# algbio/founderblockgraphs

Hardware: AMD Instinct MI355X
Metric: MSA columns segmented/sec (higher is better)
Workload: dtype u32

## Files before the change

founderblockgraphs_amd/csrc/ctx.hip:

```cpp
#include "fbg_internal.h"
#include <chrono>
#include <stdarg.h>
#include <stdio.h>
#include <ctype.h>
#include <string.h>
#include <algorithm>
#include <atomic>
#include <thread>
#include <vector>

static std::string g_global_err;

int fbg_fail(fbg_ctx *ctx, int code, const char *fmt, ...)
{
    char buf[1024];
    va_list ap;
    va_start(ap, fmt);
    vsnprintf(buf, sizeof(buf), fmt, ap);
    va_end(ap);
    if (ctx) ctx->err = buf; else g_global_err = buf;
    return code;
}

int fbg_reserve(fbg_ctx *ctx, DevBuf &b, size_t bytes, std::vector<DevBuf *> *owner, bool accounted)
// ... 160 lines not shown
    {"no_aux_stream", &FbgOptions::no_aux_stream},
    {"rank_no_threshold", &FbgOptions::rank_no_threshold},
    {"dp_literal", &FbgOptions::dp_literal},
    {"dp_wave", &FbgOptions::dp_wave},
    {"dp_safe_window", &FbgOptions::dp_safe_window},
    {"dp_tile", &FbgOptions::dp_tile},
    {"pure_scan", &FbgOptions::pure_scan},
    {"gapped_rank", &FbgOptions::gapped_rank},
    {"part_tricks_off", &FbgOptions::part_tricks_off},
    {"msd_sample_bins", &FbgOptions::msd_sample_bins},
    {"msd_min_force", &FbgOptions::msd_min_force},
    {"msd_probe", &FbgOptions::msd_probe},
    {"msd_xcd", &FbgOptions::msd_xcd},
    {"rank_no_lean", &FbgOptions::rank_no_lean},
    {"no_stream_upload", &FbgOptions::no_stream_upload},
    {"span_scan", &FbgOptions::span_scan},
    {"span_key_flags", &FbgOptions::span_key_flags},
    {"span_slow_split", &FbgOptions::span_slow_split},
    {"poison", &FbgOptions::poison},
    {"dpw_matrix", &FbgOptions::dpw_matrix},
    {"dp_chain1", &FbgOptions::dp_chain1},
    {"msd_ext", &FbgOptions::msd_ext},
    {"rows_wave", &FbgOptions::rows_wave},
};

struct InfoKey { const char *name; int64_t (*get)(const fbg_ctx &); };
static const InfoKey g_info_keys[] = {
    {"grs_threshold", [](const fbg_ctx &c) -> int64_t { return c.grs_t; }},
    {"grs_redone", [](const fbg_ctx &c) -> int64_t { return (int64_t)c.grs_redone; }},
    {"dp_kind", [](const fbg_ctx &c) -> int64_t { return c.dp_kind; }},
    {"msd_decline", [](const fbg_ctx &c) -> int64_t { return c.diag.msd_decline; }},
    {"pass1_ahead", [](const fbg_ctx &c) -> int64_t { return c.diag.pass1_ahead; }},
    {"ext_pairs", [](const fbg_ctx &c) -> int64_t { return c.diag.ext_pairs; }},
    {"text_pairs", [](const fbg_ctx &c) -> int64_t { return c.diag.text_pairs; }},
    {"rank_lean_used", [](const fbg_ctx &c) -> int64_t { return c.diag.rank_lean_used; }},
    {"rank_lean_launched", [](const fbg_ctx &c) -> int64_t { return c.diag.rank_lean_launched; }},
    {"pairs_rb", [](const fbg_ctx &c) -> int64_t { return c.diag.pairs_rb; }},
    {"key_b", [](const fbg_ctx &c) -> int64_t { return c.key_b; }},
    {"key_K", [](const fbg_ctx &c) -> int64_t { return c.key_K; }},
    {"key_packed", [](const fbg_ctx &c) -> int64_t { return c.key_packed; }},
    {"key_compact", [](const fbg_ctx &c) -> int64_t { return c.key_compact; }},
    {"alloc_calls", [](const fbg_ctx &c) -> int64_t { return (int64_t)c.alloc_calls; }},
    {"alloc_us", [](const fbg_ctx &c) -> int64_t { return (int64_t)c.alloc_us; }},
    {"span_decline", [](const fbg_ctx &c) -> int64_t { return c.diag.sp_decline; }},
    {"span_key_flags_used", [](const fbg_ctx &c) -> int64_t { return c.ix.index_valid && c.ix.spanned() && c.ix.sp_key_flags_sorted; }},
    {"span_scan_used", [](const fbg_ctx &c) -> int64_t { return c.ix.index_valid && c.ix.spanned(); }},
    {"span_scan_work", [](const fbg_ctx &c) -> int64_t { return (int64_t)c.sp_work; }},
    {"span_groups", [](const fbg_ctx &c) -> int64_t { return (int64_t)c.sp_G; }},
    {"span_odd_groups", [](const fbg_ctx &c) -> int64_t { return (int64_t)c.sp_n_odd[0] + c.sp_n_odd[1] + c.sp_n_odd[2] + c.sp_n_odd[3]; }},
    {"span_irregular", [](const fbg_ctx &c) -> int64_t { return (int64_t)c.sp_n_irr; }},
    {"span_chain", [](const fbg_ctx &c) -> int64_t { return (int64_t)c.sp_chain_n; }},
    {"span_slow_groups", [](const fbg_ctx &c) -> int64_t { return (int64_t)c.sp_slow_n; }},
    {"index_kind", [](const fbg_ctx &c) -> int64_t { return !c.ix.index_valid ? -1 : c.ix.part_active ? 3 : c.ix.granked() ? 2 : c.ix.ranked() ? 1 : 0; }},
};

static void options_from_env(FbgOptions &o)
{
// ... 512 lines not shown
```

founderblockgraphs_amd/csrc/fbg_internal.h:

```cpp
#pragma once
#include <cstring>
#include <cstdlib>
#include <hip/hip_runtime.h>
#include <stdint.h>
#include <string>
#include <vector>
#include "../../include/fbg_hip.h"

#define FBG_WAVE 64

struct DevBuf {
    void *p = nullptr;
    size_t cap = 0;
    bool listed = false;
    template <class T> T *as() const { return reinterpret_cast<T *>(p); }
};

struct Stager {
    void *base = nullptr;
    size_t slot_bytes = 0;
    int nslots = 0;
    hipEvent_t *ev = nullptr;
    hipStream_t stream = nullptr;
};

struct StageTimer {
    hipEvent_t start = nullptr, stop = nullptr;
    bool recorded = false;
    int launches = 0;
};

struct FbgOptions {
    int64_t no_ranked = 0, no_packed = 0, force_wide = 0, full_keys = 0, no_msd_sort = 0, msd_min = -1, bp_min = -1,
            record_scatter = 0, lcp_text = 0, no_aux_stream = 0, rank_no_threshold = 0, dp_literal = 0, dp_wave = 0,
            dp_safe_window = 0, dp_tile = 0, pure_scan = 0, gapped_rank = 0, part_tricks_off = 0, msd_sample_bins = 0, msd_min_force = 0, msd_probe = 0, msd_xcd = -1, rank_no_lean = 0, no_stream_upload = 0,
            span_scan = 0, span_key_flags = 0, span_slow_split = 0, poison = 0, dpw_matrix = 0, dp_chain1 = 0, msd_ext = 1, rows_wave = 0;
};

enum class IndexKind { none, record, ranked, gapped, span };

struct IndexState {
    bool index_valid = false;
    IndexKind kind = IndexKind::none;
    bool ranked() const { return kind == IndexKind::ranked; }
    bool granked() const { return kind == IndexKind::gapped || kind == IndexKind::span; }
    bool spanned() const { return kind == IndexKind::span; }
    uint32_t *sa_ptr = nullptr;
    uint64_t *rk_keys = nullptr;
    int rk_b = 0, rk_key_bits = 0, rk_K = 0;
    int rk_layout = 0, rk_pb = 0;
    bool grs_flagged = false;
    bool sp_key_flags_sorted = false;
    bool msd_ext_valid = false;
    bool lcp_from_keys = false;
    bool grs_ties_done = false;
    uint32_t n_exc = 0;
    bool part_active = false;
    bool gpart = false;
    int part = 0, nparts = 1;
    uint64_t part_count = 0;
    uint64_t part_T = 0;
    uint32_t part_gmin = 0;
};

struct BuildDiag {
    int64_t msd_decline = -1;
    int pass1_ahead = 0;
    int64_t ext_pairs = -1, text_pairs = -1;
    int rank_lean_launched = 0;
    int rank_lean_used = 0;
    int pairs_rb = -1;
    int sp_decline = 0;
};

struct SortExtras {
    const uint64_t *ebits = nullptr;
    const uint32_t *payload = nullptr;
    bool key_flags = false;
};

struct MsdPlan;
struct fbg_ctx {
    int device = 0;
    FbgOptions opt;
    std::string err;
    hipStream_t stream = nullptr;
    bool own_stream = false;
    hipStream_t aux = nullptr;
    hipEvent_t aux_fork = nullptr, aux_join = nullptr;
    bool aux_pending = false;
    Stager stager;
// ... 40 lines not shown
    DevBuf xlist;
    DevBuf gmax, excol, xslot;
    DevBuf xbits;
    DevBuf exc_scratch;
    DevBuf exc;
    int grs_tricks_off = 0;
    uint32_t grs_ign_lo = 0, grs_ign_hi = 0;
    DevBuf gwin;
    DevBuf gbits;
    bool pairs_similar = false;
    bool grs_part_failed = false;
    uint32_t grs_t = 1;
    uint64_t grs_redone = 0;
    DevBuf sp_cells;
    DevBuf sp_flagT;
    DevBuf sp_cwin;
    DevBuf sp_tiles, sp_gstart, sp_gcol, sp_gflags, sp_rstart, sp_rid, sp_gplo, sp_gphi, sp_gval, sp_odd, sp_irr, sp_chain, sp_slow, sp_mins;
    uint32_t sp_chain_n = 0, sp_slow_n = 0;
    uint64_t sp_G = 0, sp_R = 0, sp_n_irr = 0, sp_work = 0;
    uint32_t sp_n_odd[4] = {0, 0, 0, 0}, sp_odd_cap = 0;

    DevBuf keysA, keysB, valsA, valsB, grp, flags, list, tie_list, big_groups, tmp, small, scalars;
    DevBuf msd_ext;
    DevBuf kargs;
    alignas(16) unsigned char kargs_host[512];
    DevBuf msd_w, msd_v;
    DevBuf dp_a, dp_b, dp_c, dp_d, dp_e, dp_f, dp_g, dp_h, io_a, io_b, io_c, io_d;
    DevBuf bt_up, bt_dep;
    DevBuf ps_a, ps_b, ps_c, ps_d, ps_e, ps_f, ps_g, ps_h;
};

int fbg_fail(fbg_ctx *ctx, int code, const char *fmt, ...);
#define FBG_HIP_TRY(ctx, expr)                                                              \
    do {                                                                                    \
        hipError_t e_ = (expr);                                                             \
        if (e_ != hipSuccess)                                                               \
            return fbg_fail((ctx), e_ == hipErrorOutOfMemory ? FBG_ERR_OOM : FBG_ERR_HIP,   \
                            "%s failed: %s (%s:%d)", #expr, hipGetErrorString(e_), __FILE__, \
                            __LINE__);                                                      \
    } while (0)
#define FBG_TRY(expr)                \
    do {                             \
        int rc_ = (expr);            \
        if (rc_ != FBG_OK) return rc_; \
    } while (0)

// ... 99 lines not shown
```

founderblockgraphs_amd/csrc/rank_common.h:

```cpp
#pragma once
#include "fbg_internal.h"
#include "text_cmp.h"

#define RS_TG 4

__device__ __forceinline__ uint32_t rs_key_lcp(uint64_t a, uint64_t c, int b, int key_bits)
{
    const uint64_t d = a ^ c;
    const uint32_t bits = (uint32_t)(__clzll((long long)d) - (64 - key_bits));
    const uint32_t inv_b = (65536u + (uint32_t)b - 1) / (uint32_t)b;
    return (bits * inv_b) >> 16;
}

struct RankArgs {
    uint32_t magic32;
    uint64_t magic64;
    uint64_t *keys;
    uint32_t *vals;
    uint64_t pmask;
    int pb;
    const uint8_t *T;
    uint64_t N, n;
    uint64_t Ntext;
    uint64_t own_lo, own_hi;
    int first_part, last_part;
    int part_mode;
    int values_only;
    uint32_t row_len;
    uint32_t g_min;
    int b, key_bits, K, reversed;
    uint32_t *gmax;
    uint32_t *cand;
    uint32_t *blk_count;
    uint32_t region;
    uint32_t *ties;
    uint32_t *tie_count;
    uint32_t tie_region;
    uint2 *pairs;
    int pair_codes;
    unsigned long long *pair_stats;
    uint32_t *pair_count;
    uint32_t *pm;
    uint32_t *big;
    unsigned long long *counters;
};

struct Slot {
    uint64_t key;
    uint64_t pos;
    uint32_t col;
    uint32_t rem;
};

__device__ __forceinline__ uint32_t rs_col_of_rem(const RankArgs &a, uint32_t rem)
{
    return rem == 0 ? (uint32_t)a.n : (a.reversed ? rem - 1 : (uint32_t)a.n - rem);
}
template <int L> struct PosT { typedef uint32_t type; };
template <> struct PosT<FBG_SLOTS_WIDE> { typedef uint64_t type; };
template <int L> __device__ __forceinline__ uint64_t rs_key(const RankArgs &a, uint64_t k) { return a.keys[k] >> a.pb; }
template <int L> __device__ __forceinline__ uint64_t rs_pos_of(const RankArgs &a, uint64_t w, uint32_t v)
{
    if (L == FBG_SLOTS_PACKED) return w & a.pmask;
    if (L == FBG_SLOTS_WIDE) return ((w & a.pmask) << 32) | v;
    return v;
}
template <int L> __device__ __forceinline__ uint64_t rs_pos(const RankArgs &a, uint64_t k)
{
// ... 159 lines not shown
    const uint32_t lp = has_prev ? min(min(rs_key_lcp(kp, key, a.b, a.key_bits), rem), mrp) : 0u;
    const uint32_t ln = has_next ? min(min(rs_key_lcp(key, kn, a.b, a.key_bits), rem), mrn) : 0u;
    const uint32_t g = max(lp, ln) + 1;
    if (g >= a.g_min || rem <= 64) rs_update(a, rs_col_of_rem(a, rem), g);
}


static inline int rs_layout(const KeyGeom &g) { return g.packed ? FBG_SLOTS_PACKED : g.wide ? FBG_SLOTS_WIDE : FBG_SLOTS_PAIRS; }

static inline void rs_args_init(fbg_ctx *ctx, RankArgs &a, uint64_t *keys, uint32_t *vals, uint64_t slots, int layout, int pb, int b,
                         int key_bits, int K)
{
    a.keys = keys; a.vals = vals; a.T = ctx->text.as<uint8_t>();
    a.pb = layout != FBG_SLOTS_PAIRS ? pb : 0; a.pmask = layout != FBG_SLOTS_PAIRS ? (1ull << pb) - 1 : 0;
    a.N = slots; a.Ntext = ctx->N; a.n = ctx->n; a.row_len = (uint32_t)(ctx->n + 1);
    a.own_lo = 0; a.own_hi = slots; a.first_part = a.last_part = 1; a.part_mode = 0; a.values_only = 0;
    a.magic32 = (uint32_t)((1ull << 32) / (ctx->n + 1));
    a.magic64 = ~0ull / (ctx->n + 1);
    a.b = b; a.key_bits = key_bits; a.K = K; a.reversed = ctx->reversed;
    a.gmax = ctx->gmax.as<uint32_t>();
    a.cand = nullptr; a.pm = nullptr; a.blk_count = nullptr; a.region = 0;
    a.ties = nullptr; a.tie_count = nullptr; a.tie_region = 0; a.pairs = nullptr; a.pair_count = nullptr; a.pair_codes = 0;
    a.pair_stats = nullptr;
    a.big = ctx->big_groups.as<uint32_t>();
    a.counters = ctx->scalars.as<unsigned long long>() + 32;
    a.g_min = 0;
}
```

founderblockgraphs_amd/csrc/rank_scan.hip:

```cpp
#include <algorithm>
#include <cstring>
#include <vector>
#include "fbg_internal.h"
#include "text_cmp.h"
#include <rocprim/rocprim.hpp>

#include "rank_common.h"

#define RS_ITEMS 4
#define RS_THREADS 256
#define RS_CHUNK (RS_THREADS * RS_ITEMS)

template <int L, bool PLAIN> __global__ __launch_bounds__(RS_THREADS) __attribute__((amdgpu_waves_per_eu(7, 8))) void k_rank_scan(RankArgs a)
{
    __shared__ uint64_t skey[RS_CHUNK + 2 * RS_HALO];
    __shared__ uint32_t srem[RS_CHUNK + 2 * RS_HALO];
    __shared__ uint16_t sq[RS_CHUNK];
    __shared__ uint32_t sqn, s_cand_n, s_tie_n;
    const int lane = threadIdx.x & 63;
    const uint64_t nchunks = (a.own_hi - a.own_lo + RS_CHUNK - 1) / RS_CHUNK;
    if (threadIdx.x == 0) { s_cand_n = 0; s_tie_n = 0; }
    uint64_t w[RS_ITEMS + 1];
    uint32_t v[RS_ITEMS + 1];
    const int my_i = RS_HALO + RS_ITEMS * (int)threadIdx.x;
// ... 174 lines not shown

#define RL_EV_LO 3
#define RL_EV_HI 60
#define RL_EV (RL_EV_HI - RL_EV_LO + 1)
#define RL_THREADS 256
#define RL_WAVES (RL_THREADS / 64)
#define RL_LIST 128

struct LeanArgs {
    const uint64_t *keys;
    const uint8_t *ext;
    uint64_t own_lo, own_hi;
    uint32_t per_wave, pmask;
    int pb;
    float inv_row_len, eps, one_minus_eps, near_end;
};

__device__ __forceinline__ uint32_t rl_from_next(uint32_t v) { return (uint32_t)__builtin_amdgcn_update_dpp(0, (int)v, 0x130, 0xf, 0xf, false); }
__device__ __forceinline__ uint32_t rl_lanes_below(unsigned long long m)
{
    return __builtin_amdgcn_mbcnt_hi((uint32_t)(m >> 32), __builtin_amdgcn_mbcnt_lo((uint32_t)m, 0u));
}

__device__ __attribute__((noinline)) void rl_noted(const RankArgs &a, const uint2 *list, uint32_t n, uint32_t *s_pair_n)
{
    const int lane = threadIdx.x & 63;
    uint32_t base = 0;
    if (lane == 0) base = atomicAdd(s_pair_n, n);
    base = __shfl(base, 0, 64);
    if ((uint32_t)lane < n && base + (uint32_t)lane < a.tie_region) a.pairs[(size_t)blockIdx.x * a.tie_region + base + lane] = list[lane];
}

__device__ __attribute__((noinline)) void rl_queued(const RankArgs &a, const uint32_t *list, uint32_t n, uint32_t *s_cand_n, uint32_t *s_tie_n)
{
    const int lane = threadIdx.x & 63;
    bool want_cand = false, want_tie = false;
    uint64_t k = 0;
    if ((uint32_t)lane < n) {
        k = list[lane];
        const int64_t base = (int64_t)k - RS_HALO;
        const int lo_i = (int)max((int64_t)0, (int64_t)a.own_lo - base);
        const int hi_i = (int)min((int64_t)(2 * RS_HALO + 1), (int64_t)a.own_hi - base);
        const RsWordView view{a.keys + base, &a, lo_i, hi_i};
        rank_scan_slow(a, view, RS_HALO, lo_i, hi_i, k, want_cand, want_tie);
    }
    rs_append(want_cand, s_cand_n, a.cand, a.region, (uint32_t)k);
    rs_append(want_tie, s_tie_n, a.ties, a.tie_region, (uint32_t)k);
}

template <class E> __device__ __forceinline__ void rl_shift(E *list, uint32_t &n)
{
    const int lane = threadIdx.x & 63;
    const uint32_t rest = n - 64;
    if ((uint32_t)lane < rest) { const E v = list[64 + lane]; list[lane] = v; }
    n = rest;
}

__global__ __launch_bounds__(RL_THREADS) __attribute__((amdgpu_waves_per_eu(8, 8))) void k_rank_scan_lean(const RankArgs *__restrict__ ap, LeanArgs f)
{
    __shared__ uint2 s_note[RL_WAVES][RL_LIST];
    __shared__ uint32_t s_queue[RL_WAVES][RL_LIST];
    __shared__ uint32_t s_cand_n, s_tie_n, s_pair_n;
    const int lane = threadIdx.x & 63;
    const int wv = __builtin_amdgcn_readfirstlane((int)(threadIdx.x >> 6));
    if (threadIdx.x == 0) { s_cand_n = 0; s_tie_n = 0; s_pair_n = 0; }
    __syncthreads();
    uint2 *my_note = s_note[wv];
    uint32_t *my_queue = s_queue[wv];
    uint32_t nn = 0, nq = 0;
    const uint32_t own_lo = (uint32_t)f.own_lo, own_hi = (uint32_t)f.own_hi;
    const uint32_t wlo = own_lo + ((uint32_t)blockIdx.x * RL_WAVES + (uint32_t)wv) * f.per_wave;
    const uint32_t whi = min(own_hi, wlo + f.per_wave);
    const unsigned long long EVM = ((1ull << (RL_EV_HI + 1)) - 1) & ~((1ull << RL_EV_LO) - 1);
    const unsigned long long RNG = ~(1ull << 63);
    const uint64_t *__restrict__ keys = f.keys;
    const uint8_t *__restrict__ ext = f.ext;
    auto row_slot = [&](uint32_t k0) -> uint32_t { return min(max(k0 - RL_EV_LO + (uint32_t)lane, own_lo), own_hi - 1); };
    uint64_t xnext = wlo < whi ? keys[row_slot(wlo)] : 0ull;
    uint32_t enext = ext && wlo < whi ? ext[row_slot(wlo)] : 0u;
    for (uint32_t k0 = wlo; k0 < whi; k0 += RL_EV) {
        const uint64_t x = xnext;
        const uint32_t ex = enext;
        if (k0 + RL_EV < whi) {
            const uint32_t kn = row_slot(k0 + RL_EV);
            xnext = keys[kn];
            if (ext) enext = ext[kn];
        }
        const uint32_t slot = k0 - RL_EV_LO + (uint32_t)lane;
// ... 23 lines not shown
                const unsigned long long LONG = TIE & ~(PH | (PH << 1));
                const unsigned long long ADJL = ((LONG >> 1) | (LONG << 1)) & ~TIE;
                SS = EVM & PH & ~(NE | (NE >> 1) | R1 | (R1 << 1) | (R2 << 1) | R2 | (R1 >> 1) | (E << 2) | (E >> 2));
                const unsigned long long QP = EVM & PH & ~SS;
                const unsigned long long RUN = R1 | (R1 << 1) | ((PH & R2) << 2) | ((PH >> 1) & R2);
                Q = QP | (QP << 1) | (EVM & (LONG | ADJL | (~TIE & (RUN | NE))));
            }
            if (SS) {
                uint32_t cx = 0, cy = 0;
                if (ext) {
                    const uint32_t d = (ex ^ rl_from_next(ex)) & 255u;
                    const uint32_t c = d ? (uint32_t)(__builtin_clz(d) - 24) >> 1 : 4u;
                    cx = c << 30; cy = (c >> 2) << 30;
                }
                if ((SS >> lane) & 1ull) my_note[nn + rl_lanes_below(SS)] = make_uint2((lo & f.pmask) | cx, (lo_n & f.pmask) | cy);
                nn += (uint32_t)__popcll(SS);
            }
            if (Q) {
                if ((Q >> lane) & 1ull) my_queue[nq + rl_lanes_below(Q)] = slot;
                nq += (uint32_t)__popcll(Q);
            }
        }
        while (nq >= 64) { rl_queued(*ap, my_queue, 64, &s_cand_n, &s_tie_n); rl_shift(my_queue, nq); }
        if (nn >= 64) { rl_noted(*ap, my_note, 64, &s_pair_n); rl_shift(my_note, nn); }
    }
    if (nn) rl_noted(*ap, my_note, nn, &s_pair_n);
    if (nq) rl_queued(*ap, my_queue, nq, &s_cand_n, &s_tie_n);
    __syncthreads();
    if (threadIdx.x == 0) { ap->blk_count[blockIdx.x] = s_cand_n; ap->tie_count[blockIdx.x] = s_tie_n; ap->pair_count[blockIdx.x] = s_pair_n; }
}

static bool rs_lean_setup(const RankArgs &a, int pb, unsigned blocks, LeanArgs *f)
{
    const uint64_t own = a.own_hi - a.own_lo, waves = (uint64_t)blocks * RL_WAVES;
    f->per_wave = (uint32_t)(((own + waves - 1) / waves + RL_EV - 1) / RL_EV * RL_EV);
    f->keys = a.keys; f->ext = nullptr; f->own_lo = a.own_lo; f->own_hi = a.own_hi; f->pmask = (uint32_t)a.pmask; f->pb = pb;
    const double L = (double)a.row_len;
    const double delta = (ldexp(1.0, pb - 25) + ldexp(1.0, pb - 22) + 2.0) / L + 1e-6;
    f->inv_row_len = (float)(1.0 / L);
    f->eps = (float)(2.0 * delta);
    f->one_minus_eps = 1.0f - f->eps;
    f->near_end = (float)(1.0 - 65.0 / L - delta);
    return 2.0 * delta < 0.01 && pb <= 31 && a.own_hi < (1ull << 31);
}

template <int L> __global__ __launch_bounds__(256) void k_tie_simple(RankArgs a)
{
    const uint32_t have = a.tie_count[blockIdx.x];
    if (have > a.tie_region) { if (threadIdx.x == 0) a.counters[1] = 1; return; }
    for (uint32_t e = threadIdx.x; e < have; e += blockDim.x) {
        const uint64_t h = a.ties[(size_t)blockIdx.x * a.tie_region + e];
        uint64_t key[RS_TG], pos[RS_TG];
// ... 99 lines not shown
    __syncthreads();
    if (threadIdx.x < 64 && sh[threadIdx.x]) atomicAdd(&hist[threadIdx.x], sh[threadIdx.x]);
    if (threadIdx.x == 0) {
        atomicAdd(&counters[2], (unsigned long long)sties);
        atomicAdd(&counters[3], (unsigned long long)min((uint64_t)256, N - (uint64_t)blockIdx.x * 1024 * 256));
    }
}

__global__ void k_count_unfilled(const uint32_t *__restrict__ gmax, uint64_t n, uint32_t g_min, int reversed,
                                 unsigned long long *__restrict__ counters)
{
    const uint64_t x = (uint64_t)blockIdx.x * blockDim.x + threadIdx.x;
    const uint64_t rem = reversed ? x + 1 : n - x;
    const bool miss = x < n && rem > 64 && gmax[x] < g_min;
    const unsigned long long mask = __ballot(miss);
    if ((threadIdx.x & 63) == 0 && mask) atomicAdd(&counters[1 + 3], (unsigned long long)__popcll(mask));
}

__global__ void k_cand_compact(const uint32_t *__restrict__ regions, const uint32_t *__restrict__ counts,
                               const uint32_t *__restrict__ offsets, uint32_t region, uint32_t *__restrict__ out)
{
    const uint32_t c = counts[blockIdx.x] < region ? counts[blockIdx.x] : region, o = offsets[blockIdx.x];
    for (uint32_t i = threadIdx.x; i < c; i += blockDim.x) out[o + i] = regions[(size_t)blockIdx.x * region + i];
}

#define RS_BIG_GROUPS 1024
#define RS_BIG_MEMBERS 8192
template <int L> __global__ void k_tie_groups(RankArgs a, uint64_t T, int by_list)
{
    const uint64_t t = (uint64_t)blockIdx.x * blockDim.x + threadIdx.x;
    if (t >= T) return;
    const uint64_t k0 = by_list ? (uint64_t)a.cand[t] : a.own_lo + t;
    const uint64_t key = rs_key<L>(a, k0);
    if (k0 > a.own_lo && rs_key<L>(a, k0 - 1) == key) return;
    if (k0 + 1 >= a.own_hi || rs_key<L>(a, k0 + 1) != key) return;
    uint32_t s = 1;
    while (k0 + s < a.own_hi && s <= RS_BIG_MEMBERS && rs_key<L>(a, k0 + s) == key) s++;
    if (s > 64) {
        if (s > RS_BIG_MEMBERS) { a.counters[1] = 1; return; }
        const unsigned long long e = atomicAdd(&a.counters[5], 1ull);
        if (e >= RS_BIG_GROUPS) { a.counters[1] = 1; return; }
        a.big[2 * e] = (uint32_t)k0;
        a.big[2 * e + 1] = s;
        return;
    }
    typedef typename PosT<L>::type pos_t;
// ... 105 lines not shown
    isa[p] = (uint32_t)k;
    pl[p] = rs_slot_lcp<L>(a, k);
    pr[p] = rs_slot_lcp<L>(a, k + 1);
}

template <int L> __global__ void k_runs(RankArgs a, uint64_t T)
{
    const uint64_t t = (uint64_t)blockIdx.x * blockDim.x + threadIdx.x;
    if (t >= T) return;
    const uint64_t k0 = a.cand[t];
    const uint32_t col = rs_col<L>(a, k0);
    if (col == a.n) return;
    if (k0 > a.own_lo && rs_col<L>(a, k0 - 1) == col) return;
    const uint64_t lo_slot = a.first_part ? a.own_lo : 0, hi_slot = a.last_part ? a.own_hi : a.N;
    uint64_t ks = k0;
    while (ks > lo_slot && rs_col<L>(a, ks - 1) == col) ks--;
    if (ks == 0 && !a.first_part) { a.counters[1] = 1; return; }
    uint32_t run = rs_slot_lcp<L>(a, ks);
    uint64_t s = ks;
    for (;;) {
        if (s >= k0 && s < a.own_hi) a.pm[t + (s - k0)] = run;
        if (s + 1 >= hi_slot || rs_col<L>(a, s + 1) != col) break;
        s++;
        run = min(run, rs_slot_lcp<L>(a, s));
    }
    if (s + 1 == a.N && !a.last_part) { a.counters[1] = 1; return; }
    uint32_t rmin = 0xffffffffu;
    for (;; s--) {
        rmin = min(rmin, rs_slot_lcp<L>(a, s + 1));
        if (s >= k0 && s < a.own_hi) rs_update(a, col, max(a.pm[t + (s - k0)], rmin) + 1);
        if (s == ks || s <= k0) break;
    }
}

struct FinishArgs {
    const uint32_t *gmax;
    uint64_t n, x0, x1;
    int mode, disable_tricks;
    uint64_t *out;
};

__global__ void k_rank_finish(FinishArgs a)
{
    const uint64_t x = a.x0 + (uint64_t)blockIdx.x * blockDim.x + threadIdx.x;
    if (x >= a.x1) return;
    const unsigned long long g = a.gmax[x];
    if (a.mode == FBG_SCAN_V) {
        a.out[x] = g <= x + 1 ? x + 1 - g : x + 1;
        return;
    }
    unsigned long long fx = x;
    const bool any_active = a.disable_tricks || x != 0;
    if (any_active && g > 0) {
        const unsigned long long gg = x + g;
        const unsigned long long fi = gg > a.n ? (a.disable_tricks ? a.n : a.n - 1) : gg - 1;
// ... 33 lines not shown
    } while (0)

static int rs_fork(fbg_ctx *ctx)
{
    if (!ctx->aux) {
        FBG_HIP_TRY(ctx, hipStreamCreateWithFlags(&ctx->aux, hipStreamNonBlocking));
        FBG_HIP_TRY(ctx, hipEventCreateWithFlags(&ctx->aux_fork, hipEventDisableTiming));
        FBG_HIP_TRY(ctx, hipEventCreateWithFlags(&ctx->aux_join, hipEventDisableTiming));
    }
    FBG_HIP_TRY(ctx, hipEventRecord(ctx->aux_fork, ctx->stream));
    FBG_HIP_TRY(ctx, hipStreamWaitEvent(ctx->aux, ctx->aux_fork, 0));
    ctx->aux_pending = true;
    return FBG_OK;
}
static int rs_join(fbg_ctx *ctx)
{
    if (!ctx->aux_pending) return FBG_OK;
    ctx->aux_pending = false;
    FBG_HIP_TRY(ctx, hipEventRecord(ctx->aux_join, ctx->aux));
    FBG_HIP_TRY(ctx, hipStreamWaitEvent(ctx->stream, ctx->aux_join, 0));
    return FBG_OK;
}

static int rs_order_candidates(fbg_ctx *ctx, RankArgs &a, int layout, uint64_t T, int *launches)
{
    hipStream_t st = ctx->stream;
    FBG_TRY(fbg_reserve(ctx, ctx->dp_a, T * 4));
    FBG_TRY(fbg_reserve(ctx, ctx->dp_b, T * 4));
    uint32_t *sorted = ctx->dp_a.as<uint32_t>();
    uint32_t *flat = ctx->dp_e.as<uint32_t>();
    FBG_TRY(rs_with_tmp(ctx, [&](void *tmp, size_t &bytes) {
        return rocprim::radix_sort_keys(tmp, bytes, flat, sorted, (size_t)T, 0u, 32u, st);
    }));
    a.cand = sorted;
    a.pm = ctx->dp_b.as<uint32_t>();
    RS_LAUNCH(k_tie_groups, layout, dim3(fbg_blocks(T, 64)), dim3(64), st, a, T, 1);
    RS_LAUNCH(k_tie_big, layout, dim3(RS_BIG_GROUPS), dim3(256), st, a, 0);
    *launches += 3;
    return FBG_OK;
}

static int rs_classify(fbg_ctx *ctx, RankArgs &a, int layout, uint64_t *T_out, int *launches)
{
    hipStream_t st = ctx->stream;
    const uint64_t own = a.own_hi - a.own_lo;
    const unsigned rs_blocks = fbg_blocks(own, RS_CHUNK, 256 * 16);
    const uint32_t region = (uint32_t)((own / rs_blocks) / 8 + 256);
    const uint32_t tie_region = (uint32_t)((own / rs_blocks) / 6 + 256);
    FBG_TRY(fbg_reserve(ctx, ctx->list, (size_t)rs_blocks * region * 4));
    FBG_TRY(fbg_reserve(ctx, ctx->tie_list, (size_t)rs_blocks * tie_region * 4));
    FBG_TRY(fbg_reserve(ctx, ctx->big_groups, RS_BIG_GROUPS * 8));
    a.big = ctx->big_groups.as<uint32_t>();
    FBG_TRY(fbg_reserve(ctx, ctx->dp_c, (size_t)(rs_blocks + 1) * 4));
    FBG_TRY(fbg_reserve(ctx, ctx->dp_d, (size_t)(rs_blocks + 1) * 4));
    FBG_TRY(fbg_reserve(ctx, ctx->dp_f, (size_t)(rs_blocks + 1) * 4));
    FBG_HIP_TRY(ctx, hipMemsetAsync(ctx->dp_c.p, 0, (size_t)(rs_blocks + 1) * 4, st));
    FBG_HIP_TRY(ctx, hipMemsetAsync(ctx->dp_f.p, 0, (size_t)(rs_blocks + 1) * 4, st));
    a.cand = ctx->list.as<uint32_t>();
    a.blk_count = ctx->dp_c.as<uint32_t>(); a.region = region;
    a.ties = ctx->tie_list.as<uint32_t>();
    a.tie_count = ctx->dp_f.as<uint32_t>(); a.tie_region = tie_region;
    FBG_TRY(fbg_stage_begin(ctx, FBG_STAGE_RANK_KERNEL));
    LeanArgs lf;
    const bool lean = layout == FBG_SLOTS_PACKED && a.g_min > (uint32_t)a.K && !a.values_only && !a.part_mode && !ctx->opt.rank_no_lean &&
                      rs_lean_setup(a, a.pb, rs_blocks, &lf);
    ctx->diag.rank_lean_launched = lean ? 1 : 0;
    if (lean)
    {
        if (ctx->ix.msd_ext_valid && a.keys == ctx->keysA.as<uint64_t>() && a.b == 2 && a.pb <= 30 && a.own_lo == 0 && a.own_hi == ctx->N) {
            lf.ext = ctx->msd_ext.as<uint8_t>();
            a.pair_codes = 1;
        }
        a.pair_stats = ctx->scalars.as<unsigned long long>() + 112;
        FBG_HIP_TRY(ctx, hipMemsetAsync(a.pair_stats, 0, 2 * sizeof(unsigned long long), st));
        FBG_TRY(fbg_reserve(ctx, ctx->ps_g, (size_t)rs_blocks * tie_region * 8));
        FBG_TRY(fbg_reserve(ctx, ctx->ps_h, (size_t)rs_blocks * 4));
        a.pairs = ctx->ps_g.as<uint2>(); a.pair_count = ctx->ps_h.as<uint32_t>();
        static_assert(sizeof(RankArgs) <= sizeof(ctx->kargs_host), "room for the scan's arguments");
        FBG_TRY(fbg_reserve(ctx, ctx->kargs, sizeof(RankArgs)));
        memcpy(ctx->kargs_host, &a, sizeof(RankArgs));
        FBG_HIP_TRY(ctx, hipMemcpyAsync(ctx->kargs.p, ctx->kargs_host, sizeof(RankArgs), hipMemcpyHostToDevice, st));
        hipLaunchKernelGGL(k_rank_scan_lean, dim3(rs_blocks), dim3(RL_THREADS), 0, st, (const RankArgs *)ctx->kargs.p, lf);
    }
    else
        RS_LAUNCH_SCAN(layout, a.g_min <= (uint32_t)a.K || a.values_only, dim3(rs_blocks), st, a);
    FBG_TRY(fbg_stage_end(ctx, FBG_STAGE_RANK_KERNEL, 1));
    {
        hipStream_t ts = st;
        if (!ctx->opt.no_aux_stream) { FBG_TRY(rs_fork(ctx)); ts = ctx->aux; }
        if (lean) hipLaunchKernelGGL(k_tie_pairs, dim3(rs_blocks), dim3(256), 0, ts, a);
        RS_LAUNCH(k_tie_simple, layout, dim3(rs_blocks), dim3(256), ts, a);
    }
    *launches += 2;
    const int rc_rest = [&]() -> int {
        uint32_t *d_counts = a.blk_count, *d_offs = ctx->dp_d.as<uint32_t>();
        FBG_TRY(rs_with_tmp(ctx, [&](void *tmp, size_t &bytes) {
            return rocprim::exclusive_scan(tmp, bytes, d_counts, d_offs, 0u, (size_t)(rs_blocks + 1), rocprim::plus<uint32_t>(), st);
        }));
        uint32_t *d_max = reinterpret_cast<uint32_t *>(a.counters + 6);
        FBG_TRY(rs_with_tmp(ctx, [&](void *tmp, size_t &bytes) {
            return rocprim::reduce(tmp, bytes, d_counts, d_max, 0u, (size_t)rs_blocks, rocprim::maximum<uint32_t>(), st);
        }));
        uint32_t tot = 0, mx = 0;
        FBG_HIP_TRY(ctx, hipMemcpyAsync(&tot, d_offs + rs_blocks, 4, hipMemcpyDeviceToHost, st));
        FBG_HIP_TRY(ctx, hipMemcpyAsync(&mx, d_max, 4, hipMemcpyDeviceToHost, st));
        FBG_HIP_TRY(ctx, hipStreamSynchronize(st));
        const uint64_t T = tot;
        *T_out = T;
        if (mx > region) { *T_out = ~0ull; return rs_join(ctx); }
        if (T > 0) {
            FBG_TRY(fbg_reserve(ctx, ctx->dp_e, T * 4));
            uint32_t *flat = ctx->dp_e.as<uint32_t>();
            hipLaunchKernelGGL(k_cand_compact, dim3(rs_blocks), dim3(256), 0, st, a.cand, d_counts, d_offs, region, flat);
            FBG_TRY(rs_order_candidates(ctx, a, layout, T, launches));
        }
        return FBG_OK;
    }();
    if (rc_rest != FBG_OK) { (void)rs_join(ctx); return rc_rest; }
    return FBG_OK;
}

static int rs_pick_threshold(fbg_ctx *ctx, RankArgs &a, const uint64_t *keys, uint64_t count, const KeyGeom &geom, int *reject,
                             int *launches)
{
    *reject = 0;
    if (count <= (1u << 22)) return FBG_OK;
    hipStream_t st = ctx->stream;
    unsigned long long *cnt = a.counters;
    unsigned int *d_hist = reinterpret_cast<unsigned int *>(cnt + 8);
    FBG_HIP_TRY(ctx, hipMemsetAsync(d_hist, 0, 64 * sizeof(unsigned int), st));
    hipLaunchKernelGGL(k_tie_sample, dim3(fbg_blocks(count, 1024 * 256)), dim3(256), 0, st, keys, a.pb, count, geom.b, geom.key_bits,
                       cnt, d_hist);
    (*launches)++;
    unsigned long long hs[4];
    unsigned int hh[64];
    FBG_HIP_TRY(ctx, hipMemcpyAsync(hs, cnt, sizeof(hs), hipMemcpyDeviceToHost, st));
    FBG_HIP_TRY(ctx, hipMemcpyAsync(hh, d_hist, sizeof(hh), hipMemcpyDeviceToHost, st));
// ... 14 lines not shown
int fbg_rank_scan_try(fbg_ctx *ctx, uint64_t *keys, uint32_t *vals, const KeyGeom &geom, int *done)
{
    *done = 0;
    const uint64_t N = ctx->N, n = ctx->n;
    const int layout = rs_layout(geom);
    hipStream_t st = ctx->stream;
    FBG_TRY(fbg_stage_begin(ctx, FBG_STAGE_RANKSCAN));
    unsigned long long *cnt = ctx->scalars.as<unsigned long long>() + 32;
    int launches = 0;
    FBG_TRY(fbg_reserve(ctx, ctx->gmax, (n + 1) * 4));
    RankArgs a;
    rs_args_init(ctx, a, keys, vals, N, layout, geom.pb, geom.b, geom.key_bits, geom.K);
    uint64_t T = 0;
    FBG_HIP_TRY(ctx, hipMemsetAsync(cnt, 0, 8 * sizeof(unsigned long long), st));
    FBG_HIP_TRY(ctx, hipMemsetAsync(ctx->gmax.p, 0, (n + 1) * 4, st));
    int reject = 0;
    FBG_TRY(rs_pick_threshold(ctx, a, keys, N, geom, &reject, &launches));
    if (reject) return fbg_stage_end(ctx, FBG_STAGE_RANKSCAN, launches);
    FBG_TRY(rs_classify(ctx, a, layout, &T, &launches));
    if (T == ~0ull) return fbg_stage_end(ctx, FBG_STAGE_RANKSCAN, launches);
    if (T > 0) {
        RS_LAUNCH(k_runs, layout, dim3(fbg_blocks(T, 64)), dim3(64), st, a, T);
        launches++;
    }
    FBG_TRY(rs_join(ctx));
    unsigned long long h[5], ps[2] = {0, 0};
    if (a.g_min > 1)
        hipLaunchKernelGGL(k_count_unfilled, dim3(fbg_blocks(n, 256)), dim3(256), 0, st, a.gmax, n, a.g_min, a.reversed, cnt);
    FBG_HIP_TRY(ctx, hipMemcpyAsync(h, cnt, sizeof(h), hipMemcpyDeviceToHost, st));
    if (a.pair_stats) FBG_HIP_TRY(ctx, hipMemcpyAsync(ps, a.pair_stats, sizeof(ps), hipMemcpyDeviceToHost, st));
    FBG_HIP_TRY(ctx, hipStreamSynchronize(st));
    ctx->diag.ext_pairs = (int64_t)ps[0];
    ctx->diag.text_pairs = (int64_t)ps[1];
    launches++;
    if (h[1] != 0) return fbg_stage_end(ctx, FBG_STAGE_RANKSCAN, launches);
    if (a.g_min > 1 && h[4] != 0) {
        a.g_min = 0;
        a.values_only = 1;
        RS_LAUNCH_SCAN(layout, true, dim3(fbg_blocks(N, RS_CHUNK, 256 * 16)), st, a);
        launches++;
    }
    FBG_HIP_TRY(ctx, hipGetLastError());
    ctx->ix.n_exc = 0;
    ctx->ix.kind = IndexKind::ranked;
    ctx->diag.rank_lean_used = ctx->diag.rank_lean_launched;
    fbg_remember_slots(ctx, keys, vals, rs_layout(geom), geom);
    *done = 1;
    return fbg_stage_end(ctx, FBG_STAGE_RANKSCAN, launches);
}

__global__ void k_halo_export(const uint64_t *__restrict__ keys, const uint32_t *__restrict__ vals, uint64_t own_lo,
                              uint64_t own_hi, uint64_t ok, uint8_t *__restrict__ blob)
{
    uint64_t *bk = reinterpret_cast<uint64_t *>(blob);
    uint32_t *bv = reinterpret_cast<uint32_t *>(blob + 2 * FBG_PART_HALO * 8);
    uint64_t *tail = reinterpret_cast<uint64_t *>(blob + 2 * FBG_PART_HALO * 12);
// ... 173 lines not shown
```

Before: 60.11 million.

## Resolve coded pairs in scan, sort candidates in LDS, offload long runs to waves

Adds three rank-scan changes, all on by default. Coded suffix pairs are resolved directly inside the lean scan instead of being written out for later processing. Per-block candidate lists are bitonic-sorted in shared memory during compaction, so the global radix sort can be skipped when each block's list fits in LDS. Runs longer than a threshold are handed off from k_runs to a wave-parallel kernel that uses prefix-min scans. Together these aim to cut global sort and pair-processing work and the serial tail on long runs, at the cost of an extra kernel launch and extra atomics. Correctness relies on per-block sorted lists concatenating into a globally sorted order.

```diff
diff --git a/founderblockgraphs_amd/csrc/ctx.hip b/founderblockgraphs_amd/csrc/ctx.hip
--- a/founderblockgraphs_amd/csrc/ctx.hip
+++ b/founderblockgraphs_amd/csrc/ctx.hip
@@ -206,6 +206,12 @@
     {"dp_chain1", &FbgOptions::dp_chain1},
     {"msd_ext", &FbgOptions::msd_ext},
     {"rows_wave", &FbgOptions::rows_wave},
+    {"pairs_in_scan", &FbgOptions::pairs_in_scan},
+    {"runs_wave_min", &FbgOptions::runs_wave_min},
+    {"wave_list_cap", &FbgOptions::wave_list_cap},
+    {"cand_local_sort", &FbgOptions::cand_local_sort},
+    {"cand_lds_cap", &FbgOptions::cand_lds_cap},
+    {"cand_sort_check", &FbgOptions::cand_sort_check},
 };
 
 struct InfoKey { const char *name; int64_t (*get)(const fbg_ctx &); };
@@ -217,6 +223,9 @@
     {"pass1_ahead", [](const fbg_ctx &c) -> int64_t { return c.diag.pass1_ahead; }},
     {"ext_pairs", [](const fbg_ctx &c) -> int64_t { return c.diag.ext_pairs; }},
     {"text_pairs", [](const fbg_ctx &c) -> int64_t { return c.diag.text_pairs; }},
+    {"cand_inversions", [](const fbg_ctx &c) -> int64_t { return c.diag.cand_inversions; }},
+    {"cand_local_sorted", [](const fbg_ctx &c) -> int64_t { return c.diag.cand_local_sorted; }},
+    {"wave_runs", [](const fbg_ctx &c) -> int64_t { return c.diag.wave_runs; }},
     {"rank_lean_used", [](const fbg_ctx &c) -> int64_t { return c.diag.rank_lean_used; }},
     {"rank_lean_launched", [](const fbg_ctx &c) -> int64_t { return c.diag.rank_lean_launched; }},
     {"pairs_rb", [](const fbg_ctx &c) -> int64_t { return c.diag.pairs_rb; }},
diff --git a/founderblockgraphs_amd/csrc/fbg_internal.h b/founderblockgraphs_amd/csrc/fbg_internal.h
--- a/founderblockgraphs_amd/csrc/fbg_internal.h
+++ b/founderblockgraphs_amd/csrc/fbg_internal.h
@@ -34,7 +34,9 @@
     int64_t no_ranked = 0, no_packed = 0, force_wide = 0, full_keys = 0, no_msd_sort = 0, msd_min = -1, bp_min = -1,
             record_scatter = 0, lcp_text = 0, no_aux_stream = 0, rank_no_threshold = 0, dp_literal = 0, dp_wave = 0,
             dp_safe_window = 0, dp_tile = 0, pure_scan = 0, gapped_rank = 0, part_tricks_off = 0, msd_sample_bins = 0, msd_min_force = 0, msd_probe = 0, msd_xcd = -1, rank_no_lean = 0, no_stream_upload = 0,
-            span_scan = 0, span_key_flags = 0, span_slow_split = 0, poison = 0, dpw_matrix = 0, dp_chain1 = 0, msd_ext = 1, rows_wave = 0;
+            span_scan = 0, span_key_flags = 0, span_slow_split = 0, poison = 0, dpw_matrix = 0, dp_chain1 = 0, msd_ext = 1, rows_wave = 0,
+            pairs_in_scan = 1, runs_wave_min = 16, wave_list_cap = 0,
+            cand_local_sort = 1, cand_lds_cap = 0, cand_sort_check = 0;
 };
 
 enum class IndexKind { none, record, ranked, gapped, span };
@@ -67,6 +69,9 @@
     int64_t msd_decline = -1;
     int pass1_ahead = 0;
     int64_t ext_pairs = -1, text_pairs = -1;
+    int64_t wave_runs = -1;
+    int64_t cand_inversions = -1;
+    int cand_local_sorted = -1;
     int rank_lean_launched = 0;
     int rank_lean_used = 0;
     int pairs_rb = -1;
@@ -153,6 +158,7 @@
 
     DevBuf keysA, keysB, valsA, valsB, grp, flags, list, tie_list, big_groups, tmp, small, scalars;
     DevBuf msd_ext;
+    DevBuf wave_list;
     DevBuf kargs;
     alignas(16) unsigned char kargs_host[512];
     DevBuf msd_w, msd_v;
diff --git a/founderblockgraphs_amd/csrc/rank_common.h b/founderblockgraphs_amd/csrc/rank_common.h
--- a/founderblockgraphs_amd/csrc/rank_common.h
+++ b/founderblockgraphs_amd/csrc/rank_common.h
@@ -43,7 +43,12 @@
     uint32_t *pm;
     uint32_t *big;
     unsigned long long *counters;
-};
+    uint32_t *wl;
+    uint32_t wl_cap;
+    uint32_t runs_wave_min;
+    int pairs_in_scan;
+};
+#define RS_WAVE_LIST 1024
 
 struct Slot {
     uint64_t key;
@@ -249,6 +254,7 @@
     a.cand = nullptr; a.pm = nullptr; a.blk_count = nullptr; a.region = 0;
     a.ties = nullptr; a.tie_count = nullptr; a.tie_region = 0; a.pairs = nullptr; a.pair_count = nullptr; a.pair_codes = 0;
     a.pair_stats = nullptr;
+    a.wl = nullptr; a.wl_cap = 0; a.runs_wave_min = 0; a.pairs_in_scan = 0;
     a.big = ctx->big_groups.as<uint32_t>();
     a.counters = ctx->scalars.as<unsigned long long>() + 32;
     a.g_min = 0;
diff --git a/founderblockgraphs_amd/csrc/rank_scan.hip b/founderblockgraphs_amd/csrc/rank_scan.hip
--- a/founderblockgraphs_amd/csrc/rank_scan.hip
+++ b/founderblockgraphs_amd/csrc/rank_scan.hip
@@ -220,13 +220,30 @@
     return __builtin_amdgcn_mbcnt_hi((uint32_t)(m >> 32), __builtin_amdgcn_mbcnt_lo((uint32_t)m, 0u));
 }
 
-__device__ __attribute__((noinline)) void rl_noted(const RankArgs &a, const uint2 *list, uint32_t n, uint32_t *s_pair_n)
+__device__ __attribute__((noinline)) void rl_noted(const RankArgs &a, const uint2 *list, uint32_t n, uint32_t *s_pair_n, uint32_t *s_code_n)
 {
     const int lane = threadIdx.x & 63;
+    bool keep = (uint32_t)lane < n;
+    const uint2 p = keep ? list[lane] : make_uint2(0u, 0u);
+    if (a.pairs_in_scan) {
+        const uint32_t c = (p.x >> 30) | (((p.y >> 30) & 1u) << 2);
+        const bool coded = keep && c < 4;
+        if (coded) {
+            const uint32_t g = fbg_clamp_lcp((uint32_t)a.K + c) + 1;
+            rs_update(a, rs_col_of_rem(a, rs_rem<FBG_SLOTS_PACKED>(a, p.x & 0x3fffffffu)), g);
+            rs_update(a, rs_col_of_rem(a, rs_rem<FBG_SLOTS_PACKED>(a, p.y & 0x3fffffffu)), g);
+        }
+        keep = keep && !coded;
+        const unsigned long long cm = __ballot(coded);
+        if (lane == 0 && cm) atomicAdd(s_code_n, (uint32_t)__popcll(cm));
+    }
+    const unsigned long long mask = __ballot(keep);
+    if (!mask) return;
     uint32_t base = 0;
-    if (lane == 0) base = atomicAdd(s_pair_n, n);
-    base = __shfl(base, 0, 64);
-    if ((uint32_t)lane < n && base + (uint32_t)lane < a.tie_region) a.pairs[(size_t)blockIdx.x * a.tie_region + base + lane] = list[lane];
+    const int leader = __ffsll((long long)mask) - 1;
+    if (lane == leader) base = atomicAdd(s_pair_n, (uint32_t)__popcll(mask));
+    base = __shfl(base, leader, 64) + rl_lanes_below(mask);
+    if (keep && base < a.tie_region) a.pairs[(size_t)blockIdx.x * a.tie_region + base] = p;
 }
 
 __device__ __attribute__((noinline)) void rl_queued(const RankArgs &a, const uint32_t *list, uint32_t n, uint32_t *s_cand_n, uint32_t *s_tie_n)
@@ -258,10 +275,10 @@
 {
     __shared__ uint2 s_note[RL_WAVES][RL_LIST];
     __shared__ uint32_t s_queue[RL_WAVES][RL_LIST];
-    __shared__ uint32_t s_cand_n, s_tie_n, s_pair_n;
+    __shared__ uint32_t s_cand_n, s_tie_n, s_pair_n, s_code_n;
     const int lane = threadIdx.x & 63;
     const int wv = __builtin_amdgcn_readfirstlane((int)(threadIdx.x >> 6));
-    if (threadIdx.x == 0) { s_cand_n = 0; s_tie_n = 0; s_pair_n = 0; }
+    if (threadIdx.x == 0) { s_cand_n = 0; s_tie_n = 0; s_pair_n = 0; s_code_n = 0; }
     __syncthreads();
     uint2 *my_note = s_note[wv];
     uint32_t *my_queue = s_queue[wv];
@@ -331,12 +348,13 @@
             }
         }
         while (nq >= 64) { rl_queued(*ap, my_queue, 64, &s_cand_n, &s_tie_n); rl_shift(my_queue, nq); }
-        if (nn >= 64) { rl_noted(*ap, my_note, 64, &s_pair_n); rl_shift(my_note, nn); }
-    }
-    if (nn) rl_noted(*ap, my_note, nn, &s_pair_n);
+        if (nn >= 64) { rl_noted(*ap, my_note, 64, &s_pair_n, &s_code_n); rl_shift(my_note, nn); }
+    }
+    if (nn) rl_noted(*ap, my_note, nn, &s_pair_n, &s_code_n);
     if (nq) rl_queued(*ap, my_queue, nq, &s_cand_n, &s_tie_n);
     __syncthreads();
     if (threadIdx.x == 0) { ap->blk_count[blockIdx.x] = s_cand_n; ap->tie_count[blockIdx.x] = s_tie_n; ap->pair_count[blockIdx.x] = s_pair_n; }
+    if (threadIdx.x == 0 && s_code_n) atomicAdd(&ap->pair_stats[0], (unsigned long long)s_code_n);
 }
 
 static bool rs_lean_setup(const RankArgs &a, int pb, unsigned blocks, LeanArgs *f)
@@ -482,6 +500,38 @@
 {
     const uint32_t c = counts[blockIdx.x] < region ? counts[blockIdx.x] : region, o = offsets[blockIdx.x];
     for (uint32_t i = threadIdx.x; i < c; i += blockDim.x) out[o + i] = regions[(size_t)blockIdx.x * region + i];
+}
+
+#define RS_CAND_LDS 4096
+__global__ __launch_bounds__(256) void k_cand_sort_compact(const uint32_t *__restrict__ regions, const uint32_t *__restrict__ counts,
+                                                           const uint32_t *__restrict__ offsets, uint32_t region, uint32_t *__restrict__ out)
+{
+    __shared__ uint32_t buf[RS_CAND_LDS];
+    const uint32_t c = min(min(counts[blockIdx.x], region), (uint32_t)RS_CAND_LDS), o = offsets[blockIdx.x];
+    if (c == 0) return;
+    uint32_t P = 2;
+    while (P < c) P <<= 1;
+    for (uint32_t i = threadIdx.x; i < P; i += blockDim.x) buf[i] = i < c ? regions[(size_t)blockIdx.x * region + i] : 0xffffffffu;
+    __syncthreads();
+    for (uint32_t k = 2; k <= P; k <<= 1)
+        for (uint32_t j = k >> 1; j > 0; j >>= 1) {
+            for (uint32_t i = threadIdx.x; i < P; i += blockDim.x) {
+                const uint32_t l = i ^ j;
+                if (l > i) {
+                    const uint32_t x = buf[i], y = buf[l];
+                    if ((x > y) == ((i & k) == 0)) { buf[i] = y; buf[l] = x; }
+                }
+            }
+            __syncthreads();
+        }
+    for (uint32_t i = threadIdx.x; i < c; i += blockDim.x) out[o + i] = buf[i];
+}
+
+__global__ void k_cand_inversions(const uint32_t *__restrict__ cand, uint64_t T, unsigned long long *__restrict__ count)
+{
+    const uint64_t t = (uint64_t)blockIdx.x * blockDim.x + threadIdx.x;
+    const unsigned long long mask = __ballot(t + 1 < T && cand[t] >= cand[t + 1]);
+    if ((threadIdx.x & 63) == 0 && mask) atomicAdd(count, (unsigned long long)__popcll(mask));
 }
 
 #define RS_BIG_GROUPS 1024
@@ -633,6 +683,10 @@
         if (s >= k0 && s < a.own_hi) a.pm[t + (s - k0)] = run;
         if (s + 1 >= hi_slot || rs_col<L>(a, s + 1) != col) break;
         s++;
+        if (a.runs_wave_min && s - ks + 1 == a.runs_wave_min) {
+            const unsigned long long e = atomicAdd(&a.counters[7], 1ull);
+            if (e < a.wl_cap) { a.wl[2 * e] = (uint32_t)t; a.wl[2 * e + 1] = (uint32_t)ks; return; }
+        }
         run = min(run, rs_slot_lcp<L>(a, s));
     }
     if (s + 1 == a.N && !a.last_part) { a.counters[1] = 1; return; }
@@ -642,6 +696,47 @@
         if (s >= k0 && s < a.own_hi) rs_update(a, col, max(a.pm[t + (s - k0)], rmin) + 1);
         if (s == ks || s <= k0) break;
     }
+}
+
+template <int L> __global__ __launch_bounds__(64) void k_runs_long(RankArgs a)
+{
+    if (blockIdx.x >= a.counters[7]) return;
+    const uint64_t t = a.wl[2 * blockIdx.x], ks = a.wl[2 * blockIdx.x + 1];
+    const uint32_t lane = threadIdx.x;
+    const uint32_t col = rs_col<L>(a, ks);
+    uint64_t len = 0;
+    uint32_t carry = 0xffffffffu;
+    for (uint64_t c0 = 0;; c0 += 64) {
+        const uint64_t s = ks + c0 + lane;
+        const unsigned long long out = ~__ballot(s < a.own_hi && rs_col<L>(a, s) == col);
+        const uint32_t cnt = out ? (uint32_t)__ffsll((long long)out) - 1 : 64u;
+        uint32_t v = lane < cnt ? rs_slot_lcp<L>(a, s) : 0xffffffffu;
+        for (int d = 1; d < 64; d <<= 1) {
+            const uint32_t o = __shfl_up(v, d, 64);
+            if (lane >= (uint32_t)d) v = min(v, o);
+        }
+        v = min(v, carry);
+        if (lane < cnt) a.pm[t + c0 + lane] = v;
+        carry = __shfl(v, 63, 64);
+        len += cnt;
+        if (cnt < 64) break;
+    }
+    uint32_t best = 0;
+    carry = 0xffffffffu;
+    for (uint64_t c0 = (len - 1) / 64 * 64;; c0 -= 64) {
+        const uint64_t i = c0 + lane;
+        uint32_t v = i < len ? rs_slot_lcp<L>(a, ks + i + 1) : 0xffffffffu;
+        for (int d = 1; d < 64; d <<= 1) {
+            const uint32_t o = __shfl_down(v, d, 64);
+            if (lane + (uint32_t)d < 64) v = min(v, o);
+        }
+        v = min(v, carry);
+        if (i < len) best = max(best, max(a.pm[t + i], v) + 1);
+        carry = __shfl(v, 0, 64);
+        if (c0 == 0) break;
+    }
+    for (int d = 32; d > 0; d >>= 1) best = max(best, (uint32_t)__shfl_xor(best, d, 64));
+    if (lane == 0) rs_update(a, col, best);
 }
 
 struct FinishArgs {
@@ -721,16 +816,35 @@
     return FBG_OK;
 }
 
-static int rs_order_candidates(fbg_ctx *ctx, RankArgs &a, int layout, uint64_t T, int *launches)
+static int rs_wave_list(fbg_ctx *ctx, RankArgs &a)
+{
+    FBG_TRY(fbg_reserve(ctx, ctx->wave_list, (size_t)2 * RS_WAVE_LIST * 4));
+    a.wl = ctx->wave_list.as<uint32_t>();
+    const int64_t cap = ctx->opt.wave_list_cap;
+    a.wl_cap = cap > 0 && cap < RS_WAVE_LIST ? (uint32_t)cap : RS_WAVE_LIST;
+    a.runs_wave_min = ctx->opt.runs_wave_min > 0 ? (uint32_t)ctx->opt.runs_wave_min : 0u;
+    return FBG_OK;
+}
+
+static int rs_order_candidates(fbg_ctx *ctx, RankArgs &a, int layout, uint64_t T, bool sorted_already, int *launches)
 {
     hipStream_t st = ctx->stream;
     FBG_TRY(fbg_reserve(ctx, ctx->dp_a, T * 4));
     FBG_TRY(fbg_reserve(ctx, ctx->dp_b, T * 4));
     uint32_t *sorted = ctx->dp_a.as<uint32_t>();
     uint32_t *flat = ctx->dp_e.as<uint32_t>();
-    FBG_TRY(rs_with_tmp(ctx, [&](void *tmp, size_t &bytes) {
-        return rocprim::radix_sort_keys(tmp, bytes, flat, sorted, (size_t)T, 0u, 32u, st);
-    }));
+    if (!sorted_already)
+        FBG_TRY(rs_with_tmp(ctx, [&](void *tmp, size_t &bytes) {
+            return rocprim::radix_sort_keys(tmp, bytes, flat, sorted, (size_t)T, 0u, 32u, st);
+        }));
+    if (ctx->opt.cand_sort_check) {
+        unsigned long long *d_inv = ctx->scalars.as<unsigned long long>() + 114, inv = 0;
+        FBG_HIP_TRY(ctx, hipMemsetAsync(d_inv, 0, sizeof(inv), st));
+        hipLaunchKernelGGL(k_cand_inversions, dim3(fbg_blocks(T, 256)), dim3(256), 0, st, sorted, T, d_inv);
+        FBG_HIP_TRY(ctx, hipMemcpyAsync(&inv, d_inv, sizeof(inv), hipMemcpyDeviceToHost, st));
+        FBG_HIP_TRY(ctx, hipStreamSynchronize(st));
+        ctx->diag.cand_inversions = (int64_t)inv;
+    }
     a.cand = sorted;
     a.pm = ctx->dp_b.as<uint32_t>();
     RS_LAUNCH(k_tie_groups, layout, dim3(fbg_blocks(T, 64)), dim3(64), st, a, T, 1);
@@ -750,6 +864,7 @@
     FBG_TRY(fbg_reserve(ctx, ctx->tie_list, (size_t)rs_blocks * tie_region * 4));
     FBG_TRY(fbg_reserve(ctx, ctx->big_groups, RS_BIG_GROUPS * 8));
     a.big = ctx->big_groups.as<uint32_t>();
+    if (!a.part_mode) FBG_TRY(rs_wave_list(ctx, a));
     FBG_TRY(fbg_reserve(ctx, ctx->dp_c, (size_t)(rs_blocks + 1) * 4));
     FBG_TRY(fbg_reserve(ctx, ctx->dp_d, (size_t)(rs_blocks + 1) * 4));
     FBG_TRY(fbg_reserve(ctx, ctx->dp_f, (size_t)(rs_blocks + 1) * 4));
@@ -764,11 +879,13 @@
     const bool lean = layout == FBG_SLOTS_PACKED && a.g_min > (uint32_t)a.K && !a.values_only && !a.part_mode && !ctx->opt.rank_no_lean &&
                       rs_lean_setup(a, a.pb, rs_blocks, &lf);
     ctx->diag.rank_lean_launched = lean ? 1 : 0;
+    if (ctx->opt.cand_sort_check) ctx->diag.cand_inversions = 0;
     if (lean)
     {
         if (ctx->ix.msd_ext_valid && a.keys == ctx->keysA.as<uint64_t>() && a.b == 2 && a.pb <= 30 && a.own_lo == 0 && a.own_hi == ctx->N) {
             lf.ext = ctx->msd_ext.as<uint8_t>();
             a.pair_codes = 1;
+            a.pairs_in_scan = ctx->opt.pairs_in_scan != 0;
         }
         a.pair_stats = ctx->scalars.as<unsigned long long>() + 112;
         FBG_HIP_TRY(ctx, hipMemsetAsync(a.pair_stats, 0, 2 * sizeof(unsigned long long), st));
@@ -808,10 +925,18 @@
         *T_out = T;
         if (mx > region) { *T_out = ~0ull; return rs_join(ctx); }
         if (T > 0) {
-            FBG_TRY(fbg_reserve(ctx, ctx->dp_e, T * 4));
-            uint32_t *flat = ctx->dp_e.as<uint32_t>();
-            hipLaunchKernelGGL(k_cand_compact, dim3(rs_blocks), dim3(256), 0, st, a.cand, d_counts, d_offs, region, flat);
-            FBG_TRY(rs_order_candidates(ctx, a, layout, T, launches));
+            const int64_t cap_opt = ctx->opt.cand_lds_cap;
+            const uint32_t lds_cap = cap_opt > 0 && cap_opt < RS_CAND_LDS ? (uint32_t)cap_opt : RS_CAND_LDS;
+            const bool local = lean && ctx->opt.cand_local_sort && mx <= lds_cap;
+            ctx->diag.cand_local_sorted = local ? 1 : 0;
+            if (local) {
+                FBG_TRY(fbg_reserve(ctx, ctx->dp_a, T * 4));
+                hipLaunchKernelGGL(k_cand_sort_compact, dim3(rs_blocks), dim3(256), 0, st, a.cand, d_counts, d_offs, region, ctx->dp_a.as<uint32_t>());
+            } else {
+                FBG_TRY(fbg_reserve(ctx, ctx->dp_e, T * 4));
+                hipLaunchKernelGGL(k_cand_compact, dim3(rs_blocks), dim3(256), 0, st, a.cand, d_counts, d_offs, region, ctx->dp_e.as<uint32_t>());
+            }
+            FBG_TRY(rs_order_candidates(ctx, a, layout, T, local, launches));
         }
         return FBG_OK;
     }();
@@ -872,9 +997,10 @@
     if (T > 0) {
         RS_LAUNCH(k_runs, layout, dim3(fbg_blocks(T, 64)), dim3(64), st, a, T);
         launches++;
+        if (a.runs_wave_min) { RS_LAUNCH(k_runs_long, layout, dim3(a.wl_cap), dim3(64), st, a); launches++; }
     }
     FBG_TRY(rs_join(ctx));
-    unsigned long long h[5], ps[2] = {0, 0};
+    unsigned long long h[8], ps[2] = {0, 0};
     if (a.g_min > 1)
         hipLaunchKernelGGL(k_count_unfilled, dim3(fbg_blocks(n, 256)), dim3(256), 0, st, a.gmax, n, a.g_min, a.reversed, cnt);
     FBG_HIP_TRY(ctx, hipMemcpyAsync(h, cnt, sizeof(h), hipMemcpyDeviceToHost, st));
@@ -882,6 +1008,7 @@
     FBG_HIP_TRY(ctx, hipStreamSynchronize(st));
     ctx->diag.ext_pairs = (int64_t)ps[0];
     ctx->diag.text_pairs = (int64_t)ps[1];
+    ctx->diag.wave_runs = (int64_t)std::min(h[7], (unsigned long long)a.wl_cap);
     launches++;
     if (h[1] != 0) return fbg_stage_end(ctx, FBG_STAGE_RANKSCAN, launches);
     if (a.g_min > 1 && h[4] != 0) {
```

Result: faster. 62.82 million (median of 6 runs) (+4.5%).
